# howardlau1999/pytorch-ddp-template

Measured on AMD Instinct MI355X. Metric: samples/sec (whole node) ResNet-18/CIFAR-shape DDP, higher is better.
Workload: dtype bf16; 1 GPU; model=resnet18-cifar, global_batch=8192, image=32, num_classes=10, parallelism=dp1, hip_graph=True, optimizer=sgd+momentum(master fp32)

## Files before the change

### pytorch_ddp_template_amd/ops/csrc/conv_glds.hip

```cpp

#include <torch/extension.h>

#include "common.h"
#include "dispatch.h"

namespace cg {

typedef __bf16 bf16x8 __attribute__((ext_vector_type(8)));
typedef float f32x4 __attribute__((ext_vector_type(4)));

constexpr int BM = 256, BK = 64;
constexpr int THREADS = 512;

__device__ __forceinline__ f32x4 mfma16(bf16x8 a, bf16x8 b, f32x4 c) {
  return __builtin_amdgcn_mfma_f32_16x16x32_bf16(a, b, c, 0, 0, 0);
}

__device__ __forceinline__ int kswz(int row, int kbyte) {
  return kbyte ^ (((row >> 2) & 1) << 5);
}

struct Geom {
  int H, W, C, lgC, HO, WO, stride, pad, S, RS;
  int lgSt = 0;
};

constexpr int EPI_NONE = 0, EPI_ADD = 1, EPI_MASK = 2, EPI_ADD_MASK = 3;
constexpr int EPI_BNSTATS = 4, EPI_MASK_BNSTATS = EPI_MASK | EPI_BNSTATS;

template <int BN, bool STATS, int EPI = EPI_NONE>
__global__ __launch_bounds__(THREADS, BN == 64 ? 2 : 1)
void conv_fwd_glds_kernel(
    const __hip_bfloat16* __restrict__ x, const __hip_bfloat16* __restrict__ w,
    __hip_bfloat16* __restrict__ y, const __hip_bfloat16* __restrict__ zpad,
    int M, int N , int K , Geom g,
    float* __restrict__ stats_ws, int ws_nblocks,
    const __hip_bfloat16* __restrict__ addend,
    const __hip_bfloat16* __restrict__ out_mask,
    const float* __restrict__ bn_mean, const float* __restrict__ bn_rstd) {
  static_assert(!(STATS && EPI != EPI_NONE),
                "dgrad epilogues carry no forward stats");
  static_assert(!(EPI & EPI_BNSTATS) || EPI == EPI_MASK_BNSTATS,
                "BN-backward sums ride only with the mask, without an addend");
  __shared__ __hip_bfloat16 smem[2 * (BM + BN) * BK];

  const int tid = threadIdx.x;
  const int lane = tid & 63;
  const int wave = tid >> 6;

  long long nwg = (long long)gridDim.x * gridDim.y;
  long long bid = (long long)blockIdx.y * gridDim.x + blockIdx.x;
  {
    const long long q = nwg >> 3, r = nwg & 7;
    const int xcd = (int)(bid & 7);
    const long long o = bid >> 3;
    bid = (xcd < r ? xcd * (q + 1) : r * (q + 1) + (xcd - r) * q) + o;
  }
  const int n0 = (int)(bid % gridDim.x) * BN;
  const long long m0 = (bid / gridDim.x) * BM;
  const long long flat_id = bid;

  const int srow = (tid >> 3) & 7;
  const int schunk = lane & 7;
  constexpr int RA = BM / 64;
  constexpr int RB = BN / 64;

  long long nbase[RA];
  int hv[RA], wv[RA];
#pragma unroll
  for (int r = 0; r < RA; ++r) {
    const long long m = m0 + r * 64 + wave * 8 + srow;
    const int wo = (int)(m % g.WO);
    const long long t = m / g.WO;
    const int ho = (int)(t % g.HO);
    const long long n = t / g.HO;
    hv[r] = ho * g.stride - g.pad;
    wv[r] = wo * g.stride - g.pad;
    nbase[r] = n * g.H * (long long)g.W;
  }
  const int smask = (1 << g.lgSt) - 1;

  auto stage = [&](int buf, int kt) {
    __hip_bfloat16* sa = smem + buf * ((BM + BN) * BK);
    __hip_bfloat16* sb = sa + BM * BK;
    const int tap = (kt << 6) >> g.lgC;
    const int c0 = (kt << 6) & (g.C - 1);
    const int rt = tap / g.S, st = tap - rt * g.S;
#pragma unroll
    for (int r = 0; r < RA; ++r) {
      const int row = r * 64 + wave * 8 + srow;
      const int kk = c0 + kswz(row, schunk * 16) / 2;
      const __hip_bfloat16* src = zpad;
      const int hs = hv[r] + rt, ws = wv[r] + st;
      if ((unsigned)(hs >> g.lgSt) < (unsigned)g.H &&
          (unsigned)(ws >> g.lgSt) < (unsigned)g.W &&
          ((hs | ws) & smask) == 0)
        src = x + ((nbase[r] + (long long)(hs >> g.lgSt) * g.W +
                    (ws >> g.lgSt))
                   << g.lgC) +
              kk;
      __builtin_amdgcn_global_load_lds(
          (const __attribute__((address_space(1))) unsigned int*)src,
          (__attribute__((address_space(3))) unsigned int*)(
              sa + (r * 64 + wave * 8) * BK),
          16, 0, 0);
    }
#pragma unroll
    for (int r = 0; r < RB; ++r) {
      const int row = r * 64 + wave * 8 + srow;
      const long long kk = (long long)kt * BK + kswz(row, schunk * 16) / 2;
      __builtin_amdgcn_global_load_lds(
          (const __attribute__((address_space(1))) unsigned int*)(
              w + (long long)(n0 + row) * K + kk),
          (__attribute__((address_space(3))) unsigned int*)(
              sb + (r * 64 + wave * 8) * BK),
          16, 0, 0);
    }
  };

  constexpr int NWM = BM / 128;
  constexpr int NWN = 8 / NWM;
  constexpr int NI = BN / (16 * NWN);
  const int wm = (wave / NWN) * 128;
  const int wn = (wave % NWN) * (NI * 16);
  const int frow = lane & 15;
  const int fkb = (lane >> 4) * 16;

  f32x4 acc[8][NI];
#pragma unroll
  for (int i = 0; i < 8; ++i)
#pragma unroll
    for (int j = 0; j < NI; ++j) acc[i][j] = f32x4{0.f, 0.f, 0.f, 0.f};

  const int NT = K / BK;
  stage(0, 0);
  __syncthreads();

  int cur = 0;
  for (int kt = 0; kt < NT; ++kt) {
    if (kt + 1 < NT) stage(cur ^ 1, kt + 1);
    const __hip_bfloat16* sa = smem + cur * ((BM + BN) * BK);
    const __hip_bfloat16* sb = sa + BM * BK;
    bf16x8 bf[NI][2];
#pragma unroll
    for (int ni = 0; ni < NI; ++ni)
#pragma unroll
      for (int ks = 0; ks < 2; ++ks) {
        const int row = wn + ni * 16 + frow;
        bf[ni][ks] = *(const bf16x8*)((const char*)(sb + row * BK) +
                                      kswz(row, ks * 64 + fkb));
      }
#pragma unroll
    for (int mi = 0; mi < 8; ++mi) {
      bf16x8 af[2];
#pragma unroll
      for (int ks = 0; ks < 2; ++ks) {
        const int row = wm + mi * 16 + frow;
        af[ks] = *(const bf16x8*)((const char*)(sa + row * BK) +
                                  kswz(row, ks * 64 + fkb));
      }
#pragma unroll
      for (int ni = 0; ni < NI; ++ni) {
        acc[mi][ni] = mfma16(af[0], bf[ni][0], acc[mi][ni]);
        acc[mi][ni] = mfma16(af[1], bf[ni][1], acc[mi][ni]);
      }
    }
    __syncthreads();
    cur ^= 1;
  }

  if (STATS && stats_ws) {
#pragma unroll
    for (int ni = 0; ni < NI; ++ni) {
      float sv = 0.f, qv = 0.f;
#pragma unroll
      for (int mi = 0; mi < 8; ++mi)
#pragma unroll
        for (int reg = 0; reg < 4; ++reg) {
          const float v = acc[mi][ni][reg];
          sv += v;
          qv += v * v;
        }
      sv += __shfl_xor(sv, 16);
      qv += __shfl_xor(qv, 16);
      sv += __shfl_xor(sv, 32);
      qv += __shfl_xor(qv, 32);
      if (lane < 16) {
        const int col = n0 + wn + ni * 16 + frow;
        const long long wsrow =
            ((flat_id * NWM + wave / NWN)) % ws_nblocks;
        atomicAdd(&stats_ws[wsrow * N + col], sv);
        atomicAdd(&stats_ws[((long long)ws_nblocks + wsrow) * N + col], qv);
      }
    }
  }

  __hip_bfloat16* cs = smem;
  constexpr int CPR = BN / 8;
  constexpr int RPR = THREADS / CPR;
  constexpr int NR = BM / RPR;
  const int wrow = tid / CPR, wchunk = tid % CPR;
  constexpr bool HAS_ADD = (EPI & EPI_ADD) != 0;
  constexpr bool HAS_MASK = (EPI & EPI_MASK) != 0;
  constexpr bool HAS_BNS = (EPI & EPI_BNSTATS) != 0;
  constexpr int PF = 2;
  static_assert(NR >= PF, "epilogue prefetch deeper than the store loop");
  short8 av[PF] = {}, mv[PF] = {};
  auto epi_load = [&](int r, int slot) {
    const long long off =
        ((m0 + r * RPR + wrow) * N + n0) * 2 + wchunk * 16;
    if constexpr (HAS_ADD || HAS_BNS)
      av[slot] = *(const short8*)((const char*)addend + off);
    if constexpr (HAS_MASK)
      mv[slot] = *(const short8*)((const char*)out_mask + off);
  };
  if constexpr (EPI != EPI_NONE) {
#pragma unroll
    for (int p = 0; p < PF; ++p) epi_load(p, p);
  }
#pragma unroll
  for (int mi = 0; mi < 8; ++mi)
#pragma unroll
    for (int ni = 0; ni < NI; ++ni) {
      const int col = wn + ni * 16 + frow;
#pragma unroll
      for (int reg = 0; reg < 4; ++reg) {
        const int row = wm + mi * 16 + (lane >> 4) * 4 + reg;
        cs[row * BN + col] = f2bf(acc[mi][ni][reg]);
      }
    }
  float mu[8] = {}, rs[8] = {}, sdg[8] = {}, sdb[8] = {};
  if constexpr (HAS_BNS) {
#pragma unroll
    for (int j = 0; j < 8; ++j) {
      mu[j] = bn_mean[n0 + wchunk * 8 + j];
      rs[j] = bn_rstd[n0 + wchunk * 8 + j];
    }
  }
  __syncthreads();
  if constexpr (!HAS_BNS) {
#pragma unroll
    for (int r = 0; r < NR; ++r) {
      const int row = r * RPR + wrow;
      short8 c = *(const short8*)((const char*)(cs + row * BN) + wchunk * 16);
      if constexpr (EPI != EPI_NONE) {
        const short8 a = av[r % PF], m = mv[r % PF];
        if (r + PF < NR) epi_load(r + PF, r % PF);
#pragma unroll
        for (int j = 0; j < 8; ++j) {
          short v = c[j];
          if constexpr (HAS_ADD) v = f2bfbits(bfbits2f(v) + bfbits2f(a[j]));
          if constexpr (HAS_MASK)
            v = f2bfbits(bfbits2f(m[j]) > 0.f ? bfbits2f(v) : 0.f);
          c[j] = v;
        }
      }
      *(short8*)((char*)(y + (m0 + row) * N + n0) + wchunk * 16) = c;
    }
  } else {
    static_assert(PF == 2 && NR % PF == 0, "store loop steps by slot pairs");
    auto store_round = [&](int r, int slot) {
      const int row = r * RPR + wrow;
      short8 c = *(const short8*)((const char*)(cs + row * BN) + wchunk * 16);
      const short8 t = av[slot], m = mv[slot];
      if (r + PF < NR) epi_load(r + PF, slot);
#pragma unroll
      for (int j = 0; j < 8; ++j) {
        const float gv = bfbits2f(m[j]) > 0.f ? bfbits2f(c[j]) : 0.f;
        c[j] = f2bfbits(gv);
        sdb[j] += gv;
        sdg[j] += gv * (bfbits2f(t[j]) - mu[j]) * rs[j];
      }
      *(short8*)((char*)(y + (m0 + row) * N + n0) + wchunk * 16) = c;
    };
#pragma unroll 1
    for (int r = 0; r < NR; r += PF) {
      store_round(r, 0);
      store_round(r + 1, 1);
    }
  }

  if constexpr (HAS_BNS) {
    constexpr int P = THREADS / (2 * BN);
    constexpr int RP = RPR / P;
    static_assert(P >= 1 && RP * P == RPR, "column reduction split");
    static_assert((2 * RPR * BN + P * 2 * BN) * sizeof(float) <=
                      sizeof(smem), "reduction buffers exceed the tile LDS");
    float* red = reinterpret_cast<float*>(smem);
    float* red2 = red + 2 * RPR * BN;
    __syncthreads();
#pragma unroll
    for (int j = 0; j < 8; ++j) {
      red[wrow * BN + wchunk * 8 + j] = sdg[j];
      red[(RPR + wrow) * BN + wchunk * 8 + j] = sdb[j];
    }
    __syncthreads();
    const int ci = tid % (2 * BN), part = tid / (2 * BN);
    const int which = ci / BN, col = ci % BN;
    float s = 0.f;
#pragma unroll
    for (int i = 0; i < RP; ++i)
      s += red[(which * RPR + part * RP + i) * BN + col];
    if constexpr (P > 1) {
      red2[part * 2 * BN + ci] = s;
      __syncthreads();
      if (part != 0) return;
      s = red2[ci];
#pragma unroll
      for (int p = 1; p < P; ++p) s += red2[p * 2 * BN + ci];
    }
    const long long wsrow = flat_id % ws_nblocks;
    atomicAdd(&stats_ws[((long long)which * ws_nblocks + wsrow) * N + n0 + col],
              s);
  }
}

}

struct GldsBnStats {
  const torch::Tensor& bn_x;
  const torch::Tensor& mean;
  const torch::Tensor& rstd;
  torch::Tensor ws;
};

constexpr int kBnStatsRows = 1024;

static bool conv2d_glds_launch(const torch::Tensor& x, const torch::Tensor& w,
                               torch::Tensor& y, const torch::Tensor& zp,
                               int64_t stride, int64_t pad, float* stats_ws,
                               int ws_nblocks, int lgSt,
                               const c10::optional<torch::Tensor>& addend,
                               const c10::optional<torch::Tensor>& out_mask,
                               GldsBnStats* bns) {
  static const char* e = getenv("PDT_CONV_GLDS");
  if (e && e[0] == '0') return false;
  if (x.scalar_type() != torch::kBFloat16) return false;
  const int N_ = (int)x.size(0), H = (int)x.size(1), W = (int)x.size(2),
            C = (int)x.size(3);
  const int Kout = (int)w.size(0), R = (int)w.size(1), S = (int)w.size(2);
  if (C < 64 || (C & (C - 1))) return false;
  const int HO = (int)y.size(1), WO = (int)y.size(2);
  const int lgC = log2_exact(C);
  const long long M = (long long)N_ * HO * WO;
  const int K = R * S * C;
  if (Kout % 64) return false;
  const int BN = Kout % 256 == 0 ? 256 : Kout % 128 == 0 ? 128 : 64;
  if (M % cg::BM) return false;
  if (M / cg::BM > 2147483647LL / 8) return false;
  cg::Geom g{H, W, C, lgC, HO, WO, (int)stride, (int)pad, S, R * S, lgSt};
  auto stream = c10::hip::getCurrentHIPStream();
  dim3 grid(Kout / BN, (unsigned)(M / cg::BM));
  const int epi = (addend.has_value() ? cg::EPI_ADD : 0) |
                  (out_mask.has_value() ? cg::EPI_MASK : 0);
  for (const auto* t : {&addend, &out_mask}) {
    if (!t->has_value()) continue;
    TORCH_CHECK(!stats_ws,
                "conv glds: addend/out_mask exclude the stats epilogue");
    TORCH_CHECK((*t)->is_cuda() && (*t)->is_contiguous() &&
                    (*t)->scalar_type() == x.scalar_type() &&
                    (*t)->numel() == y.numel(),
                "conv glds: addend/out_mask must be contiguous, of dy's dtype "
                "and dx-sized");
  }
  const bf16* addp = addend.has_value() ? ptr16<bf16>(*addend) : nullptr;
  const bf16* maskp = out_mask.has_value() ? ptr16<bf16>(*out_mask) : nullptr;
  const float *meanp = nullptr, *rstdp = nullptr;
  if (bns) {
    TORCH_CHECK(epi == cg::EPI_MASK && !stats_ws,
                "conv glds: BN-backward sums need out_mask and no addend");
    TORCH_CHECK(bns->bn_x.is_cuda() && bns->bn_x.is_contiguous() &&
                    bns->bn_x.scalar_type() == x.scalar_type() &&
                    bns->bn_x.numel() == y.numel(),
                "conv glds: bn_x must be contiguous, of dy's dtype and "
                "dx-sized");
    for (const auto* t : {&bns->mean, &bns->rstd})
      TORCH_CHECK(t->is_cuda() && t->is_contiguous() &&
                      t->scalar_type() == torch::kFloat32 &&
                      t->numel() == Kout,
                  "conv glds: bn_mean/bn_rstd must be fp32 [C]");
    ws_nblocks = (int)std::min<long long>(kBnStatsRows,
                                          (long long)grid.x * grid.y);
    bns->ws = torch::zeros({2LL * ws_nblocks, Kout},
                           x.options().dtype(torch::kFloat32));
    stats_ws = bns->ws.data_ptr<float>();
    addp = ptr16<bf16>(bns->bn_x);
    meanp = bns->mean.data_ptr<float>();
    rstdp = bns->rstd.data_ptr<float>();
  }
#define CG_KERN(ST, EP)                                       \
  (BN == 256   ? &cg::conv_fwd_glds_kernel<256, ST, EP>       \
   : BN == 128 ? &cg::conv_fwd_glds_kernel<128, ST, EP>       \
               : &cg::conv_fwd_glds_kernel<64, ST, EP>)
  auto kern = bns                     ? CG_KERN(false, cg::EPI_MASK_BNSTATS)
              : stats_ws              ? CG_KERN(true, cg::EPI_NONE)
              : epi == cg::EPI_NONE   ? CG_KERN(false, cg::EPI_NONE)
              : epi == cg::EPI_ADD    ? CG_KERN(false, cg::EPI_ADD)
              : epi == cg::EPI_MASK   ? CG_KERN(false, cg::EPI_MASK)
                                      : CG_KERN(false, cg::EPI_ADD_MASK);
#undef CG_KERN
  hipLaunchKernelGGL(kern, grid, dim3(cg::THREADS), 0, stream, ptr16<bf16>(x),
                     ptr16<bf16>(w), ptr16<bf16>(y), ptr16<bf16>(zp), (int)M,
                     Kout, K, g, stats_ws, ws_nblocks, addp, maskp, meanp,
                     rstdp);
  return true;
}

bool conv2d_fwd_glds_ex(const torch::Tensor& x, const torch::Tensor& w,
                        torch::Tensor& y, const torch::Tensor& zp,
                        int64_t stride, int64_t pad, float* stats_ws,
                        int ws_nblocks, int lgSt,
                        const c10::optional<torch::Tensor>& addend,
                        const c10::optional<torch::Tensor>& out_mask) {
  return conv2d_glds_launch(x, w, y, zp, stride, pad, stats_ws, ws_nblocks,
                            lgSt, addend, out_mask, nullptr);
}

torch::Tensor conv2d_dgrad_glds_bnstats(
    const torch::Tensor& dy, const torch::Tensor& wr, torch::Tensor& dx,
    const torch::Tensor& zp, int64_t pad, int lgSt,
    const torch::Tensor& out_mask, const torch::Tensor& bn_x,
    const torch::Tensor& bn_mean, const torch::Tensor& bn_rstd) {
  GldsBnStats bns{bn_x, bn_mean, bn_rstd, torch::Tensor()};
  if (!conv2d_glds_launch(dy, wr, dx, zp, 1, pad, nullptr, 0, lgSt,
                          c10::nullopt, out_mask, &bns))
    return torch::Tensor();
  return bns.ws;
}

bool conv2d_fwd_glds(const torch::Tensor& x, const torch::Tensor& w,
                     torch::Tensor& y, const torch::Tensor& zp,
                     int64_t stride, int64_t pad, float* stats_ws,
                     int ws_nblocks) {
  return conv2d_fwd_glds_ex(x, w, y, zp, stride, pad, stats_ws, ws_nblocks,
                            0, c10::nullopt, c10::nullopt);
}
```

### pytorch_ddp_template_amd/ops/csrc/ops.cpp

```cpp

#include <torch/extension.h>

#include <vector>

torch::Tensor relu_fwd(torch::Tensor x);
torch::Tensor relu_bwd(torch::Tensor dy, torch::Tensor y);
torch::Tensor add_relu_fwd(torch::Tensor a, torch::Tensor b);
torch::Tensor add_(torch::Tensor a, torch::Tensor b);
torch::Tensor gelu_fwd(torch::Tensor x);
torch::Tensor gelu_bwd(torch::Tensor dy, torch::Tensor x);
torch::Tensor col_sum(torch::Tensor dy);
torch::Tensor transpose2d(torch::Tensor x);
torch::Tensor avgpool_global(torch::Tensor x);
torch::Tensor avgpool_global_bwd(torch::Tensor dy, int64_t H, int64_t W);
std::vector<torch::Tensor> maxpool2d_fwd(torch::Tensor x, int64_t k, int64_t s,
                                         int64_t p);
torch::Tensor maxpool2d_bwd(torch::Tensor dy, torch::Tensor idx, int64_t H,
                            int64_t W);
torch::Tensor weight_rot(torch::Tensor w);
torch::Tensor zero_stuff(torch::Tensor dy, int64_t s, int64_t opad_h,
                         int64_t opad_w);
torch::Tensor im2col(torch::Tensor x, int64_t R, int64_t S, int64_t stride,
                     int64_t pad, int64_t Kpad);
torch::Tensor bmm_nt_bf16(torch::Tensor A, torch::Tensor B,
                          c10::optional<torch::Tensor> bias, bool relu);
torch::Tensor gemm_nt_splitk_f32(torch::Tensor A, torch::Tensor B);
torch::Tensor bmm_tn_bf16(torch::Tensor A, torch::Tensor B);
std::vector<torch::Tensor> bmm_tn_bias_bf16(torch::Tensor A, torch::Tensor B);
torch::Tensor conv2d_fwd_bf16(torch::Tensor x, torch::Tensor w,
                              c10::optional<torch::Tensor> bias, int64_t stride,
                              int64_t pad, bool relu);
torch::Tensor conv2d_wgrad_bf16(torch::Tensor dy, torch::Tensor x,
                                int64_t stride, int64_t pad, int64_t R,
                                int64_t S);
torch::Tensor conv2d_dgrad_bf16(torch::Tensor dy, torch::Tensor wr,
                                int64_t stride, int64_t pad, int64_t H,
                                int64_t W,
                                c10::optional<torch::Tensor> addend,
                                c10::optional<torch::Tensor> addend_mask,
                                c10::optional<torch::Tensor> out_mask);
std::vector<torch::Tensor> conv2d_fwd_stats_bf16(
    torch::Tensor x, torch::Tensor w, c10::optional<torch::Tensor> bias,
    int64_t stride, int64_t pad, bool relu);
std::vector<torch::Tensor> conv2d_dgrad_bnstats_bf16(
    torch::Tensor dy, torch::Tensor wr, int64_t stride, int64_t pad, int64_t H,
    int64_t W, torch::Tensor out_mask, torch::Tensor bn_x,
    torch::Tensor bn_mean, torch::Tensor bn_rstd);
torch::Tensor bmm_nt_f32(torch::Tensor A, torch::Tensor B,
                         c10::optional<torch::Tensor> bias, bool relu);
torch::Tensor bmm_tn_f32(torch::Tensor A, torch::Tensor B);
torch::Tensor conv2d_fwd_f32(torch::Tensor x, torch::Tensor w,
                             c10::optional<torch::Tensor> bias, int64_t stride,
                             int64_t pad, bool relu);
torch::Tensor conv2d_wgrad_f32(torch::Tensor dy, torch::Tensor x,
                               int64_t stride, int64_t pad, int64_t R,
                               int64_t S);
std::vector<torch::Tensor> bn_fwd(torch::Tensor x, torch::Tensor gamma,
                                  torch::Tensor beta,
                                  c10::optional<torch::Tensor> running_mean,
                                  c10::optional<torch::Tensor> running_var,
                                  double momentum, double eps, bool relu);
std::vector<torch::Tensor> bn_fwd_ws(torch::Tensor x, torch::Tensor gamma,
                                     torch::Tensor beta, torch::Tensor ws,
                                     c10::optional<torch::Tensor> running_mean,
                                     c10::optional<torch::Tensor> running_var,
                                     double momentum, double eps, bool relu,
                                     c10::optional<torch::Tensor> addend);
torch::Tensor bn_infer(torch::Tensor x, torch::Tensor gamma, torch::Tensor beta,
                       torch::Tensor rmean, torch::Tensor rvar, double eps,
                       bool relu);
std::vector<torch::Tensor> bn_bwd(torch::Tensor dy, torch::Tensor x,
                                  torch::Tensor gamma, torch::Tensor mean,
                                  torch::Tensor rstd,
                                  c10::optional<torch::Tensor> y_relu);
std::vector<torch::Tensor> bn_bwd_ws(torch::Tensor dy, torch::Tensor x,
                                     torch::Tensor gamma, torch::Tensor mean,
                                     torch::Tensor rstd, torch::Tensor ws);
std::vector<torch::Tensor> layernorm_fwd(torch::Tensor x, torch::Tensor gamma,
                                         torch::Tensor beta, double eps);
std::vector<torch::Tensor> layernorm_bwd(torch::Tensor dy, torch::Tensor x,
                                         torch::Tensor gamma,
                                         torch::Tensor mean,
                                         torch::Tensor rstd);
torch::Tensor softmax_fwd(torch::Tensor x, double scale);
torch::Tensor softmax_bwd(torch::Tensor dy, torch::Tensor y, double scale);
std::vector<torch::Tensor> ce_fwd(torch::Tensor logits, torch::Tensor target);
torch::Tensor ce_bwd(torch::Tensor logits, torch::Tensor target,
                     torch::Tensor lse, torch::Tensor dloss);
torch::Tensor mse_fwd(torch::Tensor p, torch::Tensor t);
torch::Tensor mse_bwd(torch::Tensor p, torch::Tensor t, torch::Tensor dloss);
std::vector<torch::Tensor> qkv_unpack(torch::Tensor qkv, int64_t heads);
torch::Tensor qkv_pack(torch::Tensor dq, torch::Tensor dk, torch::Tensor dv,
                       int64_t N, int64_t heads);
torch::Tensor head_split(torch::Tensor x, int64_t heads);
std::vector<torch::Tensor> attn_fwd(torch::Tensor qkv, int64_t heads,
                                    double scale, bool want_p);
torch::Tensor attn_bwd(torch::Tensor qkv, torch::Tensor dout,
                       torch::Tensor out, torch::Tensor stats, int64_t heads,
                       double scale);
void sgd_step(std::vector<torch::Tensor> params,
              std::vector<torch::Tensor> grads,
              std::vector<torch::Tensor> moms,
              std::vector<torch::Tensor> masters, double lr, double momentum,
              double wd, double damp, bool nesterov,
              c10::optional<torch::Tensor> guard,
              c10::optional<torch::Tensor> skip_count,
              c10::optional<torch::Tensor> lr_tensor);
torch::Tensor l2norm_sq(std::vector<torch::Tensor> grads);
void scale_(std::vector<torch::Tensor> ts, double s);
void scale_by_tensor_(std::vector<torch::Tensor> ts, torch::Tensor s);


namespace {

bool is_bf16(const torch::Tensor& t) {
  return t.scalar_type() == torch::kBFloat16 ||
         t.scalar_type() == torch::kHalf;
}

int k_granule(const torch::Tensor& t) { return is_bf16(t) ? 8 : 4; }

torch::Tensor pad_k(const torch::Tensor& t, int mult) {
  long long K = t.size(-1);
  long long pad = (mult - K % mult) % mult;
  if (pad == 0) return t;
  return torch::constant_pad_nd(t, {0, pad});
}

bool pow2_ge(int v, int lo) {
  return v >= lo && (v & (v - 1)) == 0;
}

}

torch::Tensor gemm_nt(torch::Tensor A, torch::Tensor B,
                      c10::optional<torch::Tensor> bias, bool relu,
                      bool ) {
  TORCH_CHECK(A.scalar_type() == B.scalar_type(), "dtype mismatch");
  int g = k_granule(A);
  if (A.size(-1) % g) {
    A = pad_k(A.contiguous(), g);
    B = pad_k(B.contiguous(), g);
  }
  if (is_bf16(A)) return bmm_nt_bf16(A.contiguous(), B.contiguous(), bias, relu);
  return bmm_nt_f32(A.contiguous(), B.contiguous(), bias, relu);
}

torch::Tensor gemm_tn(torch::Tensor A, torch::Tensor B) {
  if (is_bf16(A)) return bmm_tn_bf16(A.contiguous(), B.contiguous());
  return bmm_tn_f32(A.contiguous(), B.contiguous());
}

torch::Tensor bmm_nt(torch::Tensor A, torch::Tensor B) {
  int g = k_granule(A);
  if (A.size(-1) % g) {
    A = pad_k(A.contiguous(), g);
    B = pad_k(B.contiguous(), g);
  }
  if (is_bf16(A)) return bmm_nt_bf16(A.contiguous(), B.contiguous(), {}, false);
  return bmm_nt_f32(A.contiguous(), B.contiguous(), {}, false);
}

torch::Tensor bmm_tn(torch::Tensor A, torch::Tensor B) {
  auto C = is_bf16(A) ? bmm_tn_bf16(A.contiguous(), B.contiguous())
                      : bmm_tn_f32(A.contiguous(), B.contiguous());
  return C.to(A.scalar_type());
}

torch::Tensor bmm_nn(torch::Tensor A, torch::Tensor B) {
  auto Bt = transpose2d(B.contiguous());
  return bmm_nt(A, Bt);
}


torch::Tensor conv2d_fwd(torch::Tensor x, torch::Tensor w,
                         c10::optional<torch::Tensor> bias, int64_t stride,
                         int64_t pad, bool relu) {
  int Cin = (int)x.size(3);
  int R = (int)w.size(1), S = (int)w.size(2), Kout = (int)w.size(0);
  const bool fast = is_bf16(x) ? pow2_ge(Cin, 8) : pow2_ge(Cin, 4);
  if (fast) {
    if (is_bf16(x))
      return conv2d_fwd_bf16(x.contiguous(), w.contiguous(), bias, stride, pad,
                             relu);
    return conv2d_fwd_f32(x.contiguous(), w.contiguous(), bias, stride, pad,
                          relu);
  }
  int K = R * S * Cin;
  int g = k_granule(x);
  int Kpad = (K + g - 1) / g * g;
  auto cols = im2col(x.contiguous(), R, S, stride, pad, Kpad);
  auto wf = pad_k(w.contiguous().reshape({Kout, K}), g);
  auto y = is_bf16(x) ? bmm_nt_bf16(cols, wf.contiguous(), bias, relu)
                      : bmm_nt_f32(cols, wf.contiguous(), bias, relu);
  int N = (int)x.size(0), H = (int)x.size(1), W = (int)x.size(2);
  int HO = (H + 2 * (int)pad - R) / (int)stride + 1;
  int WO = (W + 2 * (int)pad - S) / (int)stride + 1;
  return y.reshape({N, HO, WO, Kout});
}

torch::Tensor conv2d_dgrad(torch::Tensor dy, torch::Tensor w, int64_t stride,
                           int64_t pad, int64_t H, int64_t W,
                           c10::optional<torch::Tensor> addend,
                           c10::optional<torch::Tensor> addend_mask,
                           c10::optional<torch::Tensor> out_mask) {
  int R = (int)w.size(1), S = (int)w.size(2);
  TORCH_CHECK(pad <= R - 1 && pad <= S - 1, "dgrad needs pad <= kernel-1");
  auto wr = weight_rot(w.contiguous());
  int Kout = (int)dy.size(3);
  if (is_bf16(dy) ? pow2_ge(Kout, 8) : false) {
    return conv2d_dgrad_bf16(dy.contiguous(), wr, stride, pad, H, W, addend,
                             addend_mask, out_mask);
  }
  int64_t opad_h = (H + 2 * pad - R) % stride;
  int64_t opad_w = (W + 2 * pad - S) % stride;
  auto dys = stride > 1 ? zero_stuff(dy.contiguous(), stride, opad_h, opad_w)
                        : dy.contiguous();
  auto dx = conv2d_fwd(dys, wr, {}, 1, R - 1 - pad, false);
  if (addend.has_value()) {
    auto a = *addend;
    if (addend_mask.has_value())
      a = a * (addend_mask->reshape(a.sizes()) > 0).to(a.scalar_type());
    dx = dx + a.reshape(dx.sizes());
  }
  if (out_mask.has_value())
    dx = torch::where(out_mask->reshape(dx.sizes()) > 0, dx,
                      torch::zeros_like(dx));
  TORCH_CHECK(dx.size(1) == H && dx.size(2) == W,
              "dgrad shape mismatch: got ", dx.sizes(), " want H=", H, " W=",
              W, " (input H+2p-R must be divisible by stride)");
  return dx;
}

std::tuple<torch::Tensor, c10::optional<torch::Tensor>> conv2d_dgrad_bnstats(
    torch::Tensor dy, torch::Tensor w, int64_t stride, int64_t pad, int64_t H,
    int64_t W, torch::Tensor out_mask, torch::Tensor bn_x,
    torch::Tensor bn_mean, torch::Tensor bn_rstd) {
  int R = (int)w.size(1), S = (int)w.size(2);
  TORCH_CHECK(pad <= R - 1 && pad <= S - 1, "dgrad needs pad <= kernel-1");
  if (is_bf16(dy) && pow2_ge((int)dy.size(3), 8)) {
    auto wr = weight_rot(w.contiguous());
    auto r = conv2d_dgrad_bnstats_bf16(dy.contiguous(), wr, stride, pad, H, W,
                                       out_mask, bn_x, bn_mean, bn_rstd);
    if (r.size() == 2) return {r[0], r[1]};
    return {r[0], c10::nullopt};
  }
  return {conv2d_dgrad(dy, w, stride, pad, H, W, c10::nullopt, c10::nullopt,
                       out_mask),
          c10::nullopt};
}

torch::Tensor conv2d_wgrad(torch::Tensor dy, torch::Tensor x, int64_t stride,
                           int64_t pad, int64_t R, int64_t S) {
  int Cin = (int)x.size(3);
  const bool fast = is_bf16(x) ? pow2_ge(Cin, 8) : pow2_ge(Cin, 4);
  dy = dy.contiguous();
  x = x.contiguous();
  if (fast) {
    return is_bf16(x) ? conv2d_wgrad_bf16(dy, x, stride, pad, R, S)
                      : conv2d_wgrad_f32(dy, x, stride, pad, R, S);
  }
  int K = (int)(R * S * Cin);
  int g = k_granule(x);
  int Kpad = (K + g - 1) / g * g;
  auto cols = im2col(x, R, S, stride, pad, Kpad);
  int Kout = (int)dy.size(3);
  auto dw = is_bf16(x)
                ? bmm_tn_bf16(dy.reshape({-1, Kout}).contiguous(), cols)
                : bmm_tn_f32(dy.reshape({-1, Kout}).contiguous(), cols);
  return dw.narrow(1, 0, K).reshape({Kout, R, S, Cin}).contiguous();
}

PYBIND11_MODULE(TORCH_EXTENSION_NAME, m) {
  m.def("gemm_nt", &gemm_nt, py::arg("A"), py::arg("B"),
        py::arg("bias") = c10::nullopt, py::arg("relu") = false,
        py::arg("out_f32") = false);
  m.def("gemm_tn", &gemm_tn);
  m.def("gemm_nt_splitk_f32", &gemm_nt_splitk_f32);
  m.def("gemm_tn_bias", [](torch::Tensor A, torch::Tensor B) {
    TORCH_CHECK(A.scalar_type() == torch::kBFloat16 ||
                A.scalar_type() == torch::kHalf,
                "gemm_tn_bias: 16-bit dtypes only");
    return bmm_tn_bias_bf16(A.contiguous(), B.contiguous());
  });
  m.def("bmm_nt", &bmm_nt);
  m.def("bmm_nn", &bmm_nn);
  m.def("bmm_tn", &bmm_tn);
  m.def("transpose2d", &transpose2d);
  m.def("conv2d_fwd", &conv2d_fwd, py::arg("x"), py::arg("w"),
        py::arg("bias") = c10::nullopt, py::arg("stride") = 1,
        py::arg("pad") = 0, py::arg("relu") = false);
  m.def("conv2d_dgrad", &conv2d_dgrad, py::arg("dy"), py::arg("w"),
        py::arg("stride"), py::arg("pad"), py::arg("H"), py::arg("W"),
        py::arg("addend") = c10::nullopt,
        py::arg("addend_mask") = c10::nullopt,
        py::arg("out_mask") = c10::nullopt);
  m.def("conv2d_dgrad_bnstats", &conv2d_dgrad_bnstats, py::arg("dy"),
        py::arg("w"), py::arg("stride"), py::arg("pad"), py::arg("H"),
        py::arg("W"), py::arg("out_mask"), py::arg("bn_x"),
        py::arg("bn_mean"), py::arg("bn_rstd"));
  m.def("conv2d_fwd_stats", &conv2d_fwd_stats_bf16, py::arg("x"),
        py::arg("w"), py::arg("bias") = c10::nullopt, py::arg("stride") = 1,
        py::arg("pad") = 0, py::arg("relu") = false);
  m.def("conv2d_wgrad", &conv2d_wgrad);
  m.def("relu_fwd", &relu_fwd);
  m.def("relu_bwd", &relu_bwd);
  m.def("add_relu_fwd", &add_relu_fwd);
  m.def("add_", &add_);
  m.def("gelu_fwd", &gelu_fwd);
  m.def("gelu_bwd", &gelu_bwd);
  m.def("col_sum", &col_sum);
  m.def("avgpool_global", &avgpool_global);
  m.def("avgpool_global_bwd", &avgpool_global_bwd);
  m.def("maxpool2d_fwd", &maxpool2d_fwd);
  m.def("maxpool2d_bwd", &maxpool2d_bwd);
  m.def("bn_fwd", &bn_fwd);
  m.def("bn_fwd_ws", &bn_fwd_ws, py::arg("x"), py::arg("gamma"),
        py::arg("beta"), py::arg("ws"), py::arg("running_mean"),
        py::arg("running_var"), py::arg("momentum"), py::arg("eps"),
        py::arg("relu"), py::arg("addend") = c10::nullopt);
  m.def("bn_infer", &bn_infer);
  m.def("bn_bwd", &bn_bwd, py::arg("dy"), py::arg("x"), py::arg("gamma"),
        py::arg("mean"), py::arg("rstd"), py::arg("y_relu") = c10::nullopt);
  m.def("bn_bwd_ws", &bn_bwd_ws, py::arg("dy"), py::arg("x"),
        py::arg("gamma"), py::arg("mean"), py::arg("rstd"), py::arg("ws"));
  m.def("layernorm_fwd", &layernorm_fwd);
  m.def("layernorm_bwd", &layernorm_bwd);
  m.def("softmax_fwd", &softmax_fwd);
  m.def("attn_fwd", &attn_fwd, py::arg("qkv"), py::arg("heads"),
        py::arg("scale"), py::arg("want_p") = false);
  m.def("attn_bwd", &attn_bwd);
  m.def("qkv_unpack", &qkv_unpack);
  m.def("qkv_pack", &qkv_pack);
  m.def("head_split", &head_split);
  m.def("softmax_bwd", &softmax_bwd);
  m.def("ce_fwd", &ce_fwd);
  m.def("ce_bwd", &ce_bwd);
  m.def("mse_fwd", &mse_fwd);
  m.def("mse_bwd", &mse_bwd);
  m.def("sgd_step", &sgd_step, py::arg("params"), py::arg("grads"),
        py::arg("moms"), py::arg("masters"), py::arg("lr"),
        py::arg("momentum"), py::arg("wd"), py::arg("damp"),
        py::arg("nesterov"), py::arg("guard") = py::none(),
        py::arg("skip_count") = py::none(),
        py::arg("lr_tensor") = py::none());
  m.def("l2norm_sq", &l2norm_sq);
  m.def("scale_", &scale_);
  m.def("scale_by_tensor_", &scale_by_tensor_);
  m.def("im2col", &im2col);
  m.def("weight_rot", &weight_rot);
  m.def("zero_stuff", &zero_stuff);
}
```

Before: 135,300 samples/sec.

## Add halo-tiled 3x3 conv variant reusing LDS input rows across taps

Adds a templated halo variant of the implicit-GEMM conv kernel for 3x3, stride-1, pad-1 convolutions with 64 input channels and 64-wide output tiles. Each M-tile covers whole image rows: it loads those rows plus one halo row above and below into LDS once. All nine filter taps then read from that buffer, and only the weights are double-buffered per K step. This removes the repeated im2col-style global/LDS staging of the activation tile for every tap. In exchange it uses a different LDS layout, a higher occupancy launch bound, and more template instantiations. It is gated by an eligibility check and an environment switch.

```diff
diff --git a/pytorch_ddp_template_amd/ops/csrc/conv_glds.hip b/pytorch_ddp_template_amd/ops/csrc/conv_glds.hip
--- a/pytorch_ddp_template_amd/ops/csrc/conv_glds.hip
+++ b/pytorch_ddp_template_amd/ops/csrc/conv_glds.hip
@@ -28,8 +28,13 @@
 constexpr int EPI_NONE = 0, EPI_ADD = 1, EPI_MASK = 2, EPI_ADD_MASK = 3;
 constexpr int EPI_BNSTATS = 4, EPI_MASK_BNSTATS = EPI_MASK | EPI_BNSTATS;
 
-template <int BN, bool STATS, int EPI = EPI_NONE>
-__global__ __launch_bounds__(THREADS, BN == 64 ? 2 : 1)
+constexpr int halo_pitch(int hw) { return (hw + 2 + 7) & ~7; }
+constexpr int halo_bytes(int hw) {
+  return hw ? (BM / hw + 2) * halo_pitch(hw) * BK * 2 : 0;
+}
+
+template <int BN, bool STATS, int EPI = EPI_NONE, int HW = 0>
+__global__ __launch_bounds__(THREADS, HW ? 4 : BN == 64 ? 2 : 1)
 void conv_fwd_glds_kernel(
     const __hip_bfloat16* __restrict__ x, const __hip_bfloat16* __restrict__ w,
     __hip_bfloat16* __restrict__ y, const __hip_bfloat16* __restrict__ zpad,
@@ -42,7 +47,11 @@
                 "dgrad epilogues carry no forward stats");
   static_assert(!(EPI & EPI_BNSTATS) || EPI == EPI_MASK_BNSTATS,
                 "BN-backward sums ride only with the mask, without an addend");
-  __shared__ __hip_bfloat16 smem[2 * (BM + BN) * BK];
+  static_assert(HW == 0 || (BN == 64 && BM % HW == 0 && HW % 16 == 0),
+                "halo variant: 64-wide tile, whole image rows per M-tile");
+  constexpr int HALO_ELEMS = halo_bytes(HW) / 2;
+  __shared__ __hip_bfloat16
+      smem[HW ? HALO_ELEMS + 2 * BN * BK : 2 * (BM + BN) * BK];
 
   const int tid = threadIdx.x;
   const int lane = tid & 63;
@@ -132,41 +141,126 @@
 #pragma unroll
     for (int j = 0; j < NI; ++j) acc[i][j] = f32x4{0.f, 0.f, 0.f, 0.f};
 
-  const int NT = K / BK;
-  stage(0, 0);
-  __syncthreads();
-
-  int cur = 0;
-  for (int kt = 0; kt < NT; ++kt) {
-    if (kt + 1 < NT) stage(cur ^ 1, kt + 1);
-    const __hip_bfloat16* sa = smem + cur * ((BM + BN) * BK);
-    const __hip_bfloat16* sb = sa + BM * BK;
-    bf16x8 bf[NI][2];
-#pragma unroll
-    for (int ni = 0; ni < NI; ++ni)
-#pragma unroll
-      for (int ks = 0; ks < 2; ++ks) {
-        const int row = wn + ni * 16 + frow;
-        bf[ni][ks] = *(const bf16x8*)((const char*)(sb + row * BK) +
-                                      kswz(row, ks * 64 + fkb));
-      }
-#pragma unroll
-    for (int mi = 0; mi < 8; ++mi) {
-      bf16x8 af[2];
-#pragma unroll
-      for (int ks = 0; ks < 2; ++ks) {
-        const int row = wm + mi * 16 + frow;
-        af[ks] = *(const bf16x8*)((const char*)(sa + row * BK) +
-                                  kswz(row, ks * 64 + fkb));
-      }
-#pragma unroll
-      for (int ni = 0; ni < NI; ++ni) {
-        acc[mi][ni] = mfma16(af[0], bf[ni][0], acc[mi][ni]);
-        acc[mi][ni] = mfma16(af[1], bf[ni][1], acc[mi][ni]);
-      }
-    }
+  if constexpr (HW == 0) {
+    const int NT = K / BK;
+    stage(0, 0);
     __syncthreads();
-    cur ^= 1;
+
+    int cur = 0;
+    for (int kt = 0; kt < NT; ++kt) {
+      if (kt + 1 < NT) stage(cur ^ 1, kt + 1);
+      const __hip_bfloat16* sa = smem + cur * ((BM + BN) * BK);
+      const __hip_bfloat16* sb = sa + BM * BK;
+      bf16x8 bf[NI][2];
+#pragma unroll
+      for (int ni = 0; ni < NI; ++ni)
+#pragma unroll
+        for (int ks = 0; ks < 2; ++ks) {
+          const int row = wn + ni * 16 + frow;
+          bf[ni][ks] = *(const bf16x8*)((const char*)(sb + row * BK) +
+                                        kswz(row, ks * 64 + fkb));
+        }
+#pragma unroll
+      for (int mi = 0; mi < 8; ++mi) {
+        bf16x8 af[2];
+#pragma unroll
+        for (int ks = 0; ks < 2; ++ks) {
+          const int row = wm + mi * 16 + frow;
+          af[ks] = *(const bf16x8*)((const char*)(sa + row * BK) +
+                                    kswz(row, ks * 64 + fkb));
+        }
+#pragma unroll
+        for (int ni = 0; ni < NI; ++ni) {
+          acc[mi][ni] = mfma16(af[0], bf[ni][0], acc[mi][ni]);
+          acc[mi][ni] = mfma16(af[1], bf[ni][1], acc[mi][ni]);
+        }
+      }
+      __syncthreads();
+      cur ^= 1;
+    }
+  } else {
+    constexpr int HP = halo_pitch(HW);
+    constexpr int KR = BM / HW;
+    constexpr int PPR = HP / 8;
+    constexpr int NPIECE = (KR + 2) * PPR;
+    __hip_bfloat16* sw = smem + HALO_ELEMS;
+    const int tpi = g.H / KR;
+    const int tile = (int)(m0 / BM);
+    const long long img = tile / tpi;
+    const int h0 = (tile - (int)img * tpi) * KR;
+
+    auto stage_w = [&](int buf, int kt) {
+      __hip_bfloat16* sb = sw + buf * (BN * BK);
+#pragma unroll
+      for (int r = 0; r < RB; ++r) {
+        const int row = r * 64 + wave * 8 + srow;
+        const long long kk = (long long)kt * BK + kswz(row, schunk * 16) / 2;
+        __builtin_amdgcn_global_load_lds(
+            (const __attribute__((address_space(1))) unsigned int*)(
+                w + (long long)(n0 + row) * K + kk),
+            (__attribute__((address_space(3))) unsigned int*)(
+                sb + (r * 64 + wave * 8) * BK),
+            16, 0, 0);
+      }
+    };
+    stage_w(0, 0);
+#pragma unroll
+    for (int p0 = 0; p0 < NPIECE; p0 += 8) {
+      const int pc = p0 + wave;
+      if (pc < NPIECE) {
+        const int hr = pc / PPR;
+        const int hi = h0 - 1 + hr;
+        const int wi = (pc - hr * PPR) * 8 + (lane & 7) - 1;
+        const __hip_bfloat16* src = zpad;
+        if ((unsigned)hi < (unsigned)g.H && (unsigned)wi < (unsigned)HW)
+          src = x + (((img * g.H + hi) * HW + wi) << 6) + (lane >> 3) * 8;
+        __builtin_amdgcn_global_load_lds(
+            (const __attribute__((address_space(1))) unsigned int*)src,
+            (__attribute__((address_space(3))) unsigned int*)(smem + pc * 512),
+            16, 0, 0);
+      }
+    }
+    int abase[3];
+#pragma unroll
+    for (int st = 0; st < 3; ++st) {
+      const int q = frow + st;
+      abase[st] = (wm / HW) * HP * 128 + (q >> 3) * 1024 + (q & 7) * 16 +
+                  (lane >> 4) * 128;
+    }
+    __syncthreads();
+
+#pragma unroll 1
+    for (int rt = 0; rt < 3; ++rt)
+#pragma unroll
+    for (int st = 0; st < 3; ++st) {
+      const int kt = rt * 3 + st;
+      if (kt + 1 < 9) stage_w((kt + 1) & 1, kt + 1);
+      const __hip_bfloat16* sb = sw + (kt & 1) * (BN * BK);
+      const char* ha = (const char*)smem + rt * (HP * 128) + abase[st];
+      bf16x8 bf[NI][2];
+#pragma unroll
+      for (int ni = 0; ni < NI; ++ni)
+#pragma unroll
+        for (int ks = 0; ks < 2; ++ks) {
+          const int row = wn + ni * 16 + frow;
+          bf[ni][ks] = *(const bf16x8*)((const char*)(sb + row * BK) +
+                                        kswz(row, ks * 64 + fkb));
+        }
+#pragma unroll
+      for (int mi = 0; mi < 8; ++mi) {
+        const int cpos = ((mi * 16) / HW) * HP + (mi * 16) % HW;
+        bf16x8 af[2];
+#pragma unroll
+        for (int ks = 0; ks < 2; ++ks)
+          af[ks] = *(const bf16x8*)(ha + cpos * 128 + ks * 512);
+#pragma unroll
+        for (int ni = 0; ni < NI; ++ni) {
+          acc[mi][ni] = mfma16(af[0], bf[ni][0], acc[mi][ni]);
+          acc[mi][ni] = mfma16(af[1], bf[ni][1], acc[mi][ni]);
+        }
+      }
+      __syncthreads();
+    }
   }
 
   if (STATS && stats_ws) {
@@ -325,6 +419,17 @@
 };
 
 constexpr int kBnStatsRows = 1024;
+
+bool conv_halo64_eligible(int64_t H, int64_t W, int64_t C, int64_t Kout,
+                          int64_t R, int64_t S, int64_t stride, int64_t pad) {
+  if (R != 3 || S != 3 || stride != 1 || pad != 1 || C != 64) return false;
+  if (Kout <= 0 || Kout % 64 || Kout % 128 == 0) return false;
+  if (W < 16 || W % 16 || cg::BM % W) return false;
+  const int64_t k = cg::BM / W;
+  if (k > H || H % k) return false;
+  return cg::halo_bytes((int)W) + 2 * 64 * cg::BK * 2 <=
+         2 * (cg::BM + 64) * cg::BK * 2;
+}
 
 static bool conv2d_glds_launch(const torch::Tensor& x, const torch::Tensor& w,
                                torch::Tensor& y, const torch::Tensor& zp,
@@ -388,8 +493,16 @@
     meanp = bns->mean.data_ptr<float>();
     rstdp = bns->rstd.data_ptr<float>();
   }
+  const char* eh = getenv("PDT_CONV_HALO64");
+  const bool halo = !(eh && eh[0] == '0') && lgSt == 0 && H == HO && W == WO &&
+                    conv_halo64_eligible(H, W, C, Kout, R, S, stride, pad);
+#define CG_HALO(ST, EP)                                       \
+  (W == 16   ? &cg::conv_fwd_glds_kernel<64, ST, EP, 16>      \
+   : W == 32 ? &cg::conv_fwd_glds_kernel<64, ST, EP, 32>      \
+             : &cg::conv_fwd_glds_kernel<64, ST, EP, 64>)
 #define CG_KERN(ST, EP)                                       \
-  (BN == 256   ? &cg::conv_fwd_glds_kernel<256, ST, EP>       \
+  (halo        ? CG_HALO(ST, EP)                              \
+   : BN == 256 ? &cg::conv_fwd_glds_kernel<256, ST, EP>       \
    : BN == 128 ? &cg::conv_fwd_glds_kernel<128, ST, EP>       \
                : &cg::conv_fwd_glds_kernel<64, ST, EP>)
   auto kern = bns                     ? CG_KERN(false, cg::EPI_MASK_BNSTATS)
@@ -399,6 +512,7 @@
               : epi == cg::EPI_MASK   ? CG_KERN(false, cg::EPI_MASK)
                                       : CG_KERN(false, cg::EPI_ADD_MASK);
 #undef CG_KERN
+#undef CG_HALO
   hipLaunchKernelGGL(kern, grid, dim3(cg::THREADS), 0, stream, ptr16<bf16>(x),
                      ptr16<bf16>(w), ptr16<bf16>(y), ptr16<bf16>(zp), (int)M,
                      Kout, K, g, stats_ws, ws_nblocks, addp, maskp, meanp,
diff --git a/pytorch_ddp_template_amd/ops/csrc/ops.cpp b/pytorch_ddp_template_amd/ops/csrc/ops.cpp
--- a/pytorch_ddp_template_amd/ops/csrc/ops.cpp
+++ b/pytorch_ddp_template_amd/ops/csrc/ops.cpp
@@ -46,6 +46,8 @@
     torch::Tensor dy, torch::Tensor wr, int64_t stride, int64_t pad, int64_t H,
     int64_t W, torch::Tensor out_mask, torch::Tensor bn_x,
     torch::Tensor bn_mean, torch::Tensor bn_rstd);
+bool conv_halo64_eligible(int64_t H, int64_t W, int64_t C, int64_t Kout,
+                          int64_t R, int64_t S, int64_t stride, int64_t pad);
 torch::Tensor bmm_nt_f32(torch::Tensor A, torch::Tensor B,
                          c10::optional<torch::Tensor> bias, bool relu);
 torch::Tensor bmm_tn_f32(torch::Tensor A, torch::Tensor B);
@@ -302,6 +304,9 @@
   m.def("conv2d_fwd_stats", &conv2d_fwd_stats_bf16, py::arg("x"),
         py::arg("w"), py::arg("bias") = c10::nullopt, py::arg("stride") = 1,
         py::arg("pad") = 0, py::arg("relu") = false);
+  m.def("conv_halo64_eligible", &conv_halo64_eligible, py::arg("H"),
+        py::arg("W"), py::arg("C"), py::arg("Kout"), py::arg("R"),
+        py::arg("S"), py::arg("stride"), py::arg("pad"));
   m.def("conv2d_wgrad", &conv2d_wgrad);
   m.def("relu_fwd", &relu_fwd);
   m.def("relu_bwd", &relu_bwd);
```

New measurement: 142,800 samples/sec, median of 6. 5.6% higher.
